# 10XGenomics/supernova

Measured on AMD Instinct MI355X. Metric: Gk-mers/s through count+graph at k=48, 1.2B×150bp; bit-exact counts, higher is better.
Workload: dtype u64

## Files before the change

supernova_amd/csrc/snk_graph.h:

```cpp
#pragma once
#include "snk_ctx.h"
#include "snk_kernels.h"

struct snk_graph_out {
    uint8_t* ctx;
    uint32_t* counts;
    unsigned long long* spectrum;
    uint32_t spectrum_bins;
    uint64_t n_unitigs;
    uint64_t total_bases;
    uint64_t* unitig_off;
    uint8_t* unitig_bases;
    uint32_t* unitig_group;
    uint32_t n_circles;
    uint32_t rank_rounds;
    uint64_t n_boundary;
    uint64_t n_fragments;
};

int snk_graph_sort(snk_ctx* ctx, hipStream_t st, uint32_t K, uint64_t n, snk_u128* keys_in, uint64_t* vals_in,
                   snk_u128* keys_out, uint64_t* vals_out, char* err, size_t errcap);
int snk_graph_build(snk_ctx* ctx, hipStream_t st, uint32_t K, const snk_u128* keys, const uint64_t* vals, uint64_t n,
                    uint32_t do_prune, bool want_unitigs, snk_graph_out* out, char* err, size_t errcap);

// ... 62 lines not shown
                  const uint64_t* boff, const uint8_t* fbases, const uint32_t* fgroup, snk_join_out* out, char* err, size_t errcap);
int snk_dist_answer(snk_ctx* ctx, hipStream_t st, snk_dist_graph* g, const void* d_queries, uint64_t nq, void* d_ans, char* err,
                    size_t errcap);
int snk_dist_apply(snk_ctx* ctx, hipStream_t st, snk_dist_graph* g, const void* d_qbuf, const void* d_ans, uint64_t nq,
                   const unsigned long long* d_qoff, char* err, size_t errcap);
int snk_dist_join(snk_ctx* ctx, hipStream_t st, uint32_t K, uint64_t F, const uint32_t* nk, const unsigned long long* hl_self,
                  const unsigned long long* hl_nb, const uint64_t* boff, const uint8_t* fbases, uint64_t total_fbases,
                  snk_join_out* out, char* err, size_t errcap, const uint32_t* fgroup = nullptr, const uint32_t* sfrag = nullptr,
                  uint64_t n_states = 0, uint32_t* flink_given = nullptr);
int snk_dist_links_query(snk_ctx* ctx, hipStream_t st, bool fill, const snk_frag_out* fr, const unsigned long long* d_node_off, uint32_t world,
                         unsigned long long my_end_base, unsigned long long* d_count_or_cursor, void* d_qbuf, char* err, size_t errcap);
int snk_dist_links_answer(snk_ctx* ctx, hipStream_t st, const snk_frag_out* fr, const void* d_queries, uint64_t nq, unsigned long long my_state_base,
                          uint64_t n_local_states, unsigned long long my_end_base, void* d_ans, char* err, size_t errcap);
int snk_dist_links_apply(snk_ctx* ctx, hipStream_t st, const snk_frag_out* fr, const void* d_qbuf, const void* d_ans, uint64_t nq, uint32_t** flink_out,
                         char* err, size_t errcap);

int snk_dist_links_apply_regions(snk_ctx* ctx, hipStream_t st, const snk_frag_out* fr, const void* d_qbuf, const void* d_ans, uint32_t world, uint64_t cap,
                                 const unsigned long long* counts, uint32_t** flink_out, char* err, size_t errcap);

struct snk_table;
struct snk_bl_state {
    const snk_table* tab;
    uint32_t K, rank, world, NB_total, NBl, do_prune, force_dist;
    uint4* desc;
    uint32_t nchunks, nbig;
    uint32_t* biglist;
    uint8_t *ctx, *pend, *premote;
    uint32_t *counts, *nbr, *rq;
    uint32_t* rq_idx;
    uint16_t* rq_meta;
    unsigned long long* index;
    uint64_t index_mask, n_boundary;
    unsigned long long *qcount, *qcursor;
};
int snk_bl_dist_plan(snk_ctx* ctx, hipStream_t st, snk_bl_state* B, unsigned long long* h_qcount, char* err, size_t errcap);
int snk_bl_dist_fill(snk_ctx* ctx, hipStream_t st, snk_bl_state* B, const unsigned long long* d_qoff, void* d_qbuf, char* err, size_t errcap);
int snk_bl_dist_fragments(snk_ctx* ctx, hipStream_t st, snk_bl_state* B, const unsigned long long* d_node_off, unsigned long long my_node_off,
                          snk_frag_out* out, char* err, size_t errcap);
int snk_local_graph(snk_ctx* ctx, hipStream_t st, uint32_t K, const snk_table* tab, uint32_t do_prune, bool want_unitigs,
                    bool sort_table, bool grouped, snk_graph_out* out, snk_u128** keys_final, float* ms , char* err,
                    size_t errcap);
int snk_spectrum(snk_ctx* ctx, hipStream_t st, const uint32_t* counts, uint64_t n, unsigned long long** bins_out, uint32_t* nbins_out,
                 char* err, size_t errcap);
```

supernova_amd/csrc/snk_graph.hip:

```cpp
#include <string.h>
#include <cstring>
#include <rocprim/rocprim.hpp>

#include "snk_ctx.h"
#include "snk_common.h"
#include "snk_kernels.h"
#include "snk_graph.h"
#include "snk_stages.h"

namespace {

constexpr uint32_t NONE = 0xFFFFFFFFu;
constexpr int TB = 256;

__device__ __forceinline__ snk_kmer load_key(const snk_u128* keys, uint64_t i) {
    const uint64_t* p = reinterpret_cast<const uint64_t*>(keys + i);
    snk_kmer k;
    k.lo = p[0];
    k.hi = p[1];
    return k;
}

__global__ void __launch_bounds__(TB) index_build_kernel(const snk_u128* __restrict__ keys, uint64_t n,
                                                         unsigned long long* __restrict__ tab, uint64_t mask) {
// ... 291 lines not shown
        SNK_HIP_TRY(snk_launch(sorted_check_kernel, snk_blocks(n, 256), 256, 0, st, keys_out, n, bad));
        uint32_t h_bad = 0;
        SNK_HIP_TRY(hipMemcpyAsync(&h_bad, bad, 4, hipMemcpyDeviceToHost, st));
        SNK_HIP_TRY(snk_sync(st));
        if (!h_bad) return SNK_OK;
        if (begin_bit == 0) break;
    }
    return snk_fail(SNK_E_INTERNAL, err, errcap, "retained k-mer table is not strictly ascending after the sort");
}

__global__ void __launch_bounds__(TB) rank_init_w_kernel(const uint32_t* __restrict__ link, const uint32_t* __restrict__ w,
                                                         uint64_t ns, uint32_t* __restrict__ nxt, uint32_t* __restrict__ dist,
                                                         uint32_t* __restrict__ tail) {
    uint64_t s = (uint64_t)blockIdx.x * TB + threadIdx.x;
    if (s >= ns) return;
    uint32_t l = link[s];
    if (l == NONE) { nxt[s] = NONE; dist[s] = 0; tail[s] = (uint32_t)s; }
    else { nxt[s] = l ^ 1u; dist[s] = w[l >> 1]; tail[s] = l ^ 1u; }
}
__global__ void __launch_bounds__(TB) rank_zip_kernel(const uint32_t* __restrict__ dist, const uint32_t* __restrict__ tail, uint64_t ns,
                                                      uint2* __restrict__ rk) {
    uint64_t s = (uint64_t)blockIdx.x * TB + threadIdx.x;
    if (s < ns) rk[s] = make_uint2(dist[s], tail[s]);
}

static int rank_lists_wyllie(snk_ctx* ctx, hipStream_t st, uint32_t* link, uint64_t n, const uint32_t* weights, uint8_t* circ ,
                      const uint2** rk_out, uint32_t* n_circles, uint32_t* rounds,
                      char* err, size_t errcap) {
    const uint64_t ns = 2 * n;
    uint32_t *nxt[2], *dst[2], *tl[2];
    for (int b = 0; b < 2; ++b) { G_ALLOC(nxt[b], uint32_t, ns); G_ALLOC(dst[b], uint32_t, ns); G_ALLOC(tl[b], uint32_t, ns); }
    uint32_t* flags;
    G_ALLOC(flags, uint32_t, 4);
    uint32_t* h_flags = nullptr;
    SNK_HIP_TRY(hipHostMalloc((void**)&h_flags, 16, hipHostMallocDefault));
    int max_rounds = 2;
    while ((1ull << (max_rounds - 1)) < ns) ++max_rounds;
    int cur = 0;
    uint32_t rounds_total = 0;
    for (int attempt = 0; attempt < 2; ++attempt) {
        cur = 0;
        if (weights) SNK_HIP_TRY(snk_launch(rank_init_w_kernel, snk_blocks(ns, TB), TB, 0, st, link, weights, ns, nxt[0], dst[0], tl[0]));
        else SNK_HIP_TRY(snk_launch(rank_init_kernel, snk_blocks(ns, TB), TB, 0, st, link, ns, nxt[0], dst[0], tl[0]));
        bool converged = false;
        for (int r = 0; r < max_rounds; ++r) {
            SNK_HIP_TRY(hipMemsetAsync(flags, 0, 4, st));
            SNK_HIP_TRY(snk_launch(rank_round_kernel, snk_blocks(ns, TB), TB, 0, st, nxt[cur], dst[cur], tl[cur], ns,
                                   nxt[cur ^ 1], dst[cur ^ 1], tl[cur ^ 1], flags));
            cur ^= 1;
            ++rounds_total;
            SNK_HIP_TRY(hipMemcpyAsync(h_flags, flags, 4, hipMemcpyDeviceToHost, st));
            SNK_HIP_TRY(snk_sync(st));
            if (h_flags[0] == 0) { converged = true; break; }
        }
        if (converged) break;
        if (attempt == 1) { (void)hipHostFree(h_flags); return snk_fail(SNK_E_INTERNAL, err, errcap, "unitig ranking did not converge after the circle cut"); }
        uint32_t *jump[2] = {dst[cur ^ 1], tl[cur ^ 1]};
        uint32_t* mn[2];
        G_ALLOC(mn[0], uint32_t, ns);
        G_ALLOC(mn[1], uint32_t, ns);
        SNK_HIP_TRY(snk_launch(cyc_init_kernel, snk_blocks(ns, TB), TB, 0, st, nxt[cur], link, ns, jump[0], mn[0]));
        int c2 = 0;
        for (int r = 0; r < max_rounds; ++r) {
            SNK_HIP_TRY(snk_launch(cyc_round_kernel, snk_blocks(ns, TB), TB, 0, st, jump[c2], mn[c2], ns, jump[c2 ^ 1], mn[c2 ^ 1]));
            c2 ^= 1;
        }
// ... 28 lines not shown
                                                         uint32_t* __restrict__ spl_state) {
    uint64_t s = (uint64_t)blockIdx.x * TB + threadIdx.x;
    if (s >= ns || !spl[s]) return;
    spl_state[sid[s]] = (uint32_t)s;
}
__global__ void __launch_bounds__(TB) spl_pack_kernel(const uint32_t* __restrict__ link, const uint8_t* __restrict__ spl,
                                                      const uint32_t* __restrict__ sid, uint64_t ns, unsigned long long* __restrict__ wrec) {
    uint64_t s = (uint64_t)blockIdx.x * TB + threadIdx.x;
    if (s >= ns) return;
    unsigned long long r = link[s];
    if (spl[s]) r |= ((unsigned long long)sid[s] << 32) | (1ull << 63);
    wrec[s] = r;
}
__global__ void __launch_bounds__(TB) spl_walk1_kernel(const unsigned long long* __restrict__ wrec, const uint32_t* __restrict__ spl_state,
                                                       const uint32_t* __restrict__ w, uint64_t m, uint32_t* __restrict__ rnxt,
                                                       uint32_t* __restrict__ rdist, uint32_t* __restrict__ rtail) {
    uint64_t k = (uint64_t)blockIdx.x * TB + threadIdx.x;
    if (k >= m) return;
    uint32_t cur = spl_state[k];
    unsigned long long rec = wrec[cur];
    uint32_t d = 0, nx = NONE;
    for (;;) {
        uint32_t l = (uint32_t)rec;
        if (l == NONE) { nx = NONE; break; }
        cur = l ^ 1u;
        rec = wrec[cur];
        d += w ? w[cur >> 1] : 1u;
        if (rec >> 63) { nx = (uint32_t)(rec >> 32) & 0x7FFFFFFFu; break; }
    }
    rnxt[k] = nx;
    rdist[k] = d;
    rtail[k] = cur;
}
__global__ void __launch_bounds__(TB) spl_walk2_kernel(const unsigned long long* __restrict__ wrec, const uint32_t* __restrict__ spl_state,
                                                       const uint32_t* __restrict__ w, const uint32_t* __restrict__ rdist,
                                                       const uint32_t* __restrict__ rtail, uint64_t m, uint2* __restrict__ rk) {
    uint64_t k = (uint64_t)blockIdx.x * TB + threadIdx.x;
    if (k >= m) return;
    uint32_t cur = spl_state[k];
    unsigned long long rec = wrec[cur];
    uint32_t d = rdist[k];
    const uint32_t t = rtail[k];
    for (;;) {
        rk[cur] = make_uint2(d, t);
        uint32_t l = (uint32_t)rec;
        if (l == NONE) break;
        cur = l ^ 1u;
        rec = wrec[cur];
        if (rec >> 63) break;
        d -= w ? w[cur >> 1] : 1u;
    }
}
__global__ void __launch_bounds__(TB) unranked_check_kernel(const uint2* __restrict__ rk, uint64_t ns, uint32_t* __restrict__ flag) {
    uint64_t s = (uint64_t)blockIdx.x * TB + threadIdx.x;
    if (s < ns && rk[s].y == NONE) *flag = 1u;
}

__global__ void __launch_bounds__(TB) spl_reach_kernel(const unsigned long long* __restrict__ wrec, const uint32_t* __restrict__ spl_state, uint64_t m,
                                                       uint8_t* __restrict__ reach) {
    const uint64_t k = (uint64_t)blockIdx.x * TB + threadIdx.x;
    if (k >= m) return;
    uint32_t cur = spl_state[k];
    unsigned long long rec = wrec[cur];
    for (;;) {
        reach[cur] = 1;
        const uint32_t l = (uint32_t)rec;
        if (l == NONE) break;
        cur = l ^ 1u;
        rec = wrec[cur];
        if (rec >> 63) break;
    }
}
__global__ void __launch_bounds__(TB) scyc_init_kernel(const uint32_t* __restrict__ rn_final, const uint32_t* __restrict__ rn_orig,
                                                       const uint32_t* __restrict__ spl_state, uint64_t m, uint32_t* __restrict__ jump, uint32_t* __restrict__ mn) {
    const uint64_t k = (uint64_t)blockIdx.x * TB + threadIdx.x;
    if (k >= m) return;
    const bool on = rn_final[k] != NONE;
    jump[k] = on ? rn_orig[k] : NONE;
    mn[k] = on ? spl_state[k] >> 1 : NONE;
}
__device__ __forceinline__ void cut_at(uint32_t* link, uint32_t s, uint8_t* circ, uint32_t* n_cut) {
    const uint32_t partner = link[s];
    link[s] = NONE;
    if (partner != NONE) link[partner] = NONE;
    circ[s] = 1;
    if (partner != NONE) circ[partner] = 1;
    atomicAdd(n_cut, 1u);
}
// ... 43 lines not shown
        SNK_HIP_TRY(snk_launch(scyc_init_kernel, snk_blocks(m, TB), TB, 0, st, rn_final, rn_orig, spl_state, m, jump[0], mn[0]));
        int max_rounds = 2;
        while ((1ull << (max_rounds - 1)) < m + 1) ++max_rounds;
        int c2 = 0;
        for (int r = 0; r < max_rounds; ++r) {
            SNK_HIP_TRY(snk_launch(cyc_round_kernel, snk_blocks(m, TB), TB, 0, st, jump[c2], mn[c2], m, jump[c2 ^ 1], mn[c2 ^ 1]));
            c2 ^= 1;
        }
        SNK_HIP_TRY(snk_launch(scyc_cut_kernel, snk_blocks(m, TB), TB, 0, st, mn[c2], spl_state, m, link, d_flags, circ));
    }
    {
        const uint32_t cap = 1u << 18;
        uint32_t* list;
        G_ALLOC(list, uint32_t, cap);
        SNK_HIP_TRY(snk_launch(free_circle_find_kernel, snk_blocks(ns, TB), TB, 0, st, reach, ns, (const uint32_t*)link, list, cap, d_flags + 2, d_flags + 1));
        SNK_HIP_TRY(snk_launch(cut_list_kernel, cap / TB, TB, 0, st, (const uint32_t*)list, (const uint32_t*)(d_flags + 2), cap, link, d_flags, circ));
    }
    uint32_t h[2] = {0, 0};
    SNK_HIP_TRY(hipMemcpyAsync(h, d_flags, 8, hipMemcpyDeviceToHost, st));
    SNK_HIP_TRY(snk_sync(st));
    *n_cut = h[0];
    *bad = h[1];
    return SNK_OK;
}

static int rank_lists(snk_ctx* ctx, hipStream_t st, uint32_t* link, uint64_t n, const uint32_t* weights, uint8_t* circ ,
                      const uint2** rk_out, uint32_t* n_circles, uint32_t* rounds,
                      char* err, size_t errcap) {
    const uint64_t ns = 2 * n;
    if (ns < 4096 || snk_opt_u32(ctx, SNK_OPT_rank_wyllie))
        return rank_lists_wyllie(ctx, st, link, n, weights, circ, rk_out, n_circles, rounds, err, errcap);
    uint32_t cut_total = 0;
    for (int attempt = 0; attempt < 2; ++attempt) {
    uint8_t* spl;
    uint32_t *flag32, *sid;
    G_ALLOC(spl, uint8_t, ns + 1);
    G_ALLOC(flag32, uint32_t, ns + 1);
    G_ALLOC(sid, uint32_t, ns + 1);
    SNK_HIP_TRY(hipMemsetAsync(flag32 + ns, 0, 4, st));
    const uint32_t split_mask = (1u << snk_opt_u32(ctx, SNK_OPT_split_log2)) - 1u;
    SNK_HIP_TRY(snk_launch(spl_mark_kernel, snk_blocks(ns, TB), TB, 0, st, link, ns, split_mask, spl, flag32));
    {
        size_t tb = 0;
        SNK_HIP_TRY(rocprim::exclusive_scan((void*)nullptr, tb, flag32, sid, 0u, (size_t)(ns + 1), rocprim::plus<uint32_t>(), st));
        void* tmp;
        int rc = snk_ctx_alloc(ctx, tb, &tmp, err, errcap);
        if (rc) return rc;
        SNK_HIP_TRY(rocprim::exclusive_scan(tmp, tb, flag32, sid, 0u, (size_t)(ns + 1), rocprim::plus<uint32_t>(), st));
    }
    uint32_t m32 = 0;
    SNK_HIP_TRY(hipMemcpyAsync(&m32, sid + ns, 4, hipMemcpyDeviceToHost, st));
    SNK_HIP_TRY(snk_sync(st));
    const uint64_t m = m32;
    uint32_t* spl_state = flag32;
    if (m) SNK_HIP_TRY(snk_launch(spl_collect_kernel, snk_blocks(ns, TB), TB, 0, st, spl, sid, ns, spl_state));
    uint32_t *rn[2], *rd[2], *rt[2];
    for (int b = 0; b < 2; ++b) { G_ALLOC(rn[b], uint32_t, m + 1); G_ALLOC(rd[b], uint32_t, m + 1); G_ALLOC(rt[b], uint32_t, m + 1); }
    unsigned long long* wrec;
    G_ALLOC(wrec, unsigned long long, ns);
    SNK_HIP_TRY(snk_launch(spl_pack_kernel, snk_blocks(ns, TB), TB, 0, st, link, spl, sid, ns, wrec));
    SNK_HIP_TRY(snk_launch(spl_walk1_kernel, snk_blocks(m, TB), TB, 0, st, wrec, spl_state, weights, m, rn[0], rd[0], rt[0]));
    uint32_t* rn_orig;
    G_ALLOC(rn_orig, uint32_t, m + 1);
    if (m) SNK_HIP_TRY(hipMemcpyAsync(rn_orig, rn[0], m * 4, hipMemcpyDeviceToDevice, st));
    uint32_t* flags;
    G_ALLOC(flags, uint32_t, 4);
    int max_rounds = 2;
    while ((1ull << (max_rounds - 1)) < m + 1) ++max_rounds;
    int cur = 0;
    uint32_t r_done = 0;
    uint2* rk = nullptr;
    bool converged = false, unranked = false;
    G_ALLOC(rk, uint2, ns);
    const int batch0 = (int)snk_opt_u32(ctx, SNK_OPT_rank_round_batch0);
    for (int r = 0; r < max_rounds && !converged;) {
        const int upto = r == 0 ? (batch0 < max_rounds ? batch0 : max_rounds) : max_rounds;
        SNK_HIP_TRY(hipMemsetAsync(flags, 0, 8, st));
        for (; r < upto; ++r) {
            SNK_HIP_TRY(snk_launch(rank_round_kernel, snk_blocks(m, TB), TB, 0, st, rn[cur], rd[cur], rt[cur], m, rn[cur ^ 1], rd[cur ^ 1], rt[cur ^ 1],
                                   r + 1 == upto ? flags : flags + 2));
            cur ^= 1;
            ++r_done;
        }
        SNK_HIP_TRY(hipMemsetAsync(rk, 0xFF, ns * 8, st));
        SNK_HIP_TRY(snk_launch(spl_walk2_kernel, snk_blocks(m, TB), TB, 0, st, wrec, spl_state, weights, rd[cur], rt[cur], m, rk));
        SNK_HIP_TRY(snk_launch(unranked_check_kernel, snk_blocks(ns, TB), TB, 0, st, rk, ns, flags + 1));
        uint32_t h2[2] = {0, 0};
        SNK_HIP_TRY(hipMemcpyAsync(h2, flags, 8, hipMemcpyDeviceToHost, st));
        SNK_HIP_TRY(snk_sync(st));
        converged = h2[0] == 0;
        unranked = h2[1] != 0;
    }
    if (converged && !unranked) {
        *rk_out = rk;
        *n_circles = cut_total;
        *rounds = r_done;
        return SNK_OK;
    }
    if (!circ || attempt == 1) break;
    uint32_t n_cut = 0, bad = 0;
    int rcc = cut_circles_sparse(ctx, st, link, ns, m, spl_state, wrec, rn_orig, rn[cur], converged, circ, &n_cut, &bad, err, errcap);
    if (rcc) return rcc;
    if (bad || n_cut == 0) break;
    cut_total += n_cut;
    }
    {
        uint32_t nc2 = 0;
        int rcw = rank_lists_wyllie(ctx, st, link, n, weights, circ, rk_out, &nc2, rounds, err, errcap);
        *n_circles = cut_total + nc2;
        return rcw;
    }
}

namespace {
__global__ void __launch_bounds__(TB) spl_walk1p_kernel(const unsigned long long* __restrict__ wrec, const uint32_t* __restrict__ spl_state,
                                                        const uint32_t* __restrict__ w, uint64_t k0, uint64_t cnt, uint4* __restrict__ out) {
    const uint64_t i = (uint64_t)blockIdx.x * TB + threadIdx.x;
    if (i >= cnt) return;
    uint32_t cur = spl_state[k0 + i];
    unsigned long long rec = wrec[cur];
    uint32_t d = 0, nx = NONE, steps = 1;
    for (;;) {
        const uint32_t l = (uint32_t)rec;
        if (l == NONE) { nx = NONE; break; }
        cur = l ^ 1u;
        rec = wrec[cur];
        d += w[cur >> 1];
        if (rec >> 63) { nx = (uint32_t)(rec >> 32) & 0x7FFFFFFFu; break; }
        ++steps;
    }
    out[i] = make_uint4(nx, d, cur, steps);
}
// ... 986 lines not shown
```

supernova_amd/csrc/snk_local.hip:

```cpp
#include <string.h>
#include <cstring>
#include <rocprim/rocprim.hpp>

#include <type_traits>

#include "snk_ctx.h"
#include "snk_common.h"
#include "snk_kernels.h"
#include "snk_graph.h"
#include "snk_stages.h"

namespace {

constexpr uint32_t NONE = 0xFFFFFFFFu;
constexpr unsigned long long NONE64 = ~0ull;
constexpr uint16_t NONE16 = 0xFFFFu;
constexpr int TB = 256;

struct chunk_src {
    const uint32_t* chunk_n;
    const uint32_t* chunk_base;
    const uint4* extra;
    const unsigned long long* region_off;
    uint32_t NB, n_extra, n_regions;
// ... 45 lines not shown
    } else {
        const uint4 e = cs.extra[c - cs.NB];
        bucket = e.x; off = e.y; n = e.z & 0xFFFu; region = e.z >> 12; meta = e.w;
    }
    const uint64_t base = cs.region_off[region] + off;
    desc[c] = make_uint4((uint32_t)base, n, bucket, meta);
    if (desc_src) desc_src[c] = (uint64_t)region * region_cap + off;
}
__device__ __forceinline__ chunk_t chunk_get(const uint4* __restrict__ desc, uint32_t c) {
    const uint4 d = desc[c];
    chunk_t k;
    k.base = d.x; k.n = d.y; k.bucket = d.z; k.lg = d.w >> 24; k.id = d.w & 0xFFFFFFu; k.span = 1;
    if (d.w >> 31) { k.lg = 0; k.id = 0; k.span = d.w & 0xFFFFu; }
    return k;
}

__device__ __forceinline__ snk_kmer load_key(const snk_u128* keys, uint64_t i) {
    const uint64_t* p = reinterpret_cast<const uint64_t*>(keys + i);
    snk_kmer k;
    k.lo = p[0];
    k.hi = p[1];
    return k;
}
__device__ __forceinline__ uint32_t lhash(uint64_t hi, uint64_t lo) {
    uint32_t x = (uint32_t)(hi >> 32) * 0x9E3779B1u ^ (uint32_t)hi * 0x85EBCA77u ^ (uint32_t)(lo >> 32) * 0xC2B2AE3Du ^
                 (uint32_t)lo * 0x27D4EB2Fu;
    return snk_mix32(x);
}
template <int K>
__device__ __forceinline__ uint32_t oriented_base(snk_kmer k, bool rc, int idx) {
    return rc ? (snk_kmer_base<K>(k, K - 1 - idx) ^ 3u) : snk_kmer_base<K>(k, idx);
}

template <int K, int CAP, int T, bool BIG, bool GR, int MM>
__device__ __forceinline__ void bl_prune_chunk(const uint32_t c, const uint4* __restrict__ desc, uint32_t NB, bl_shard sh, const bl_regions& rg,
                                                     const snk_u128* __restrict__ keys, const uint64_t* __restrict__ vals,
                                                     uint32_t do_prune, uint8_t* __restrict__ ctx_out,
                                                     uint32_t* __restrict__ count_out, uint8_t* __restrict__ pend_out,
                                                     uint32_t* __restrict__ nbr_out, uint32_t* __restrict__ nbnd,
                                                     uint32_t* __restrict__ biglist, uint32_t* __restrict__ nbig,
                                                     unsigned long long* __restrict__ gindex, uint64_t gmask) {
    constexpr int HT = CAP <= 256 ? 512 : 4096;
    typedef typename std::conditional<(K <= 48 && !GR), uint32_t, uint64_t>::type klo_w;
    constexpr int KLS = (K <= 48 && !GR) ? 32 : 0;
    __shared__ uint64_t khi[CAP];
    __shared__ klo_w klo[CAP];
    __shared__ uint32_t ht[HT];
    __shared__ uint32_t bcnt;
    const int tid = threadIdx.x;
    const chunk_t ch = chunk_get(desc, c);
    if (ch.n == 0) return;
    if (!BIG && ch.n > (uint32_t)CAP) {
        if (tid == 0) biglist[atomicAdd(nbig, 1u)] = c;
        return;
    }
    const uint32_t n = ch.n;
    uint64_t src = ch.base;
    if (rg.keys_r) { src = rg.desc_src[c]; keys = rg.keys_r; vals = rg.vals_r; }
    __syncthreads();
    for (int s = tid; s < HT; s += T) ht[s] = 0;
    if (tid == 0) bcnt = 0;
    constexpr int NPT = (CAP + T - 1) / T;
    uint64_t myv[NPT];
    snk_kmer kq[NPT];
#pragma unroll
    for (int q = 0; q < NPT; ++q) {
        const uint32_t i = tid + q * T;
        myv[q] = 0;
        if (i < n) {
            kq[q] = load_key(keys, src + i);
            myv[q] = vals[src + i];
        }
    }
#pragma unroll
// ... 100 lines not shown
                uint64_t wn;
                if (bit < 4) {
                    constexpr int pl = K - MM;
                    wn = pl < 32 ? ((y.hi << (2 * pl)) | (y.lo >> (64 - 2 * pl))) : (pl == 32 ? y.lo : (y.lo << (2 * pl - 64)));
                } else wn = y.hi;
                const uint32_t nkey = snk_mmer_key_top<MM>(wn);
                if (nkey < mk) mk = nkey;
                const uint32_t gb = snk_bucket_of_key(mk ^ (GR ? snk_group_mix((uint32_t)ktag) : 0u), NB);
                const uint32_t db = gb - (sh.bucket_base + ch.bucket);
                bool here = ch.span == 1 ? db == 0u : (gb >= sh.bucket_base + ch.bucket && db % sh.G == 0u && db / sh.G < ch.span);
                const bool remote = sh.NBl && gb / sh.NBl != sh.me;
                if (here && ch.lg) {
                    const snk_kmer r = snk_kmer_rc<K>(y);
                    snk_kmer cn = snk_kmer_lt(r, y) ? r : y;
                    if (GR) cn.lo |= ktag;
                    uint32_t h1, h2;
                    snk_kmer_hash_count<(K > 48) || GR>(cn, &h1, &h2);
                    here = (h2 & split_mask) == ch.id;
                }
                if (here && !(do_prune & 2u)) { if (!(do_prune & 1u)) atomicOr(&resL[th], 1u << bit); }
                else atomicOr(&resL[th], (1u << bit) | (0x100u << bit) | (remote ? (0x10000u << bit) : 0u));
            }
        }
        __syncthreads();
        const uint32_t res = resL[tid];
        keep |= res & 0xFFu;
        const uint32_t pm = (res >> 8) & 0xFFu;
        __syncthreads();
        if (!act) continue;
        const uint64_t gi = ch.base + i;
        ctx_out[gi] = (uint8_t)keep;
        pend_out[gi] = (uint8_t)pm;
        if (sh.premote) sh.premote[gi] = (uint8_t)(res >> 16);
        count_out[gi] = (uint32_t)(v >> 8);
        nbr_out[gi] = (nb0 == NONE ? 0x0FFFu : nb0) | (snk_kmer_eq(k, kr) ? 0x8000u : 0u) | ((nb1 == NONE ? 0x0FFFu : nb1) << 16);
        if (pm) {
            ++mybnd;
            if (gindex) {
                snk_kmer kk;
                kk.hi = khi[i];
                kk.lo = (uint64_t)klo[i] << KLS;
                uint32_t h1, h2;
                snk_kmer_hash2(kk, &h1, &h2);
                uint64_t slot = (((uint64_t)h1 << 32) | h2) & gmask;
                const unsigned long long ent = ((unsigned long long)h1 << 32) | (unsigned long long)(gi + 1);
                if (gindex[gmask + 1] == 0ull) {
                    bool placed = false;
                    for (uint32_t tries = 0; tries < 64; ++tries) {
                        const unsigned long long old = atomicCAS(&gindex[slot], 0ull, ent);
                        if (old == 0ull) { placed = true; break; }
                        slot = (slot + 1) & gmask;
                    }
                    if (!placed) gindex[gmask + 1] = 1ull;
                }
            }
        }
    }
    snk_wave_add(&bcnt, mybnd);
    __syncthreads();
    if (tid == 0) nbnd[c] = bcnt;
}
template <int K, int CAP, int T, bool BIG, bool GR, int MM>
__global__ void __launch_bounds__(T) bl_prune_kernel(const uint4* __restrict__ desc, uint32_t NB, bl_shard sh, bl_regions rg, const uint32_t* __restrict__ biglist_in,
                                                     uint32_t nchunks, uint32_t cpw,
                                                     const snk_u128* __restrict__ keys, const uint64_t* __restrict__ vals,
                                                     uint32_t do_prune, uint8_t* __restrict__ ctx_out,
                                                     uint32_t* __restrict__ count_out, uint8_t* __restrict__ pend_out,
                                                     uint32_t* __restrict__ nbr_out, uint32_t* __restrict__ nbnd,
                                                     uint32_t* __restrict__ biglist, uint32_t* __restrict__ nbig, const uint32_t* __restrict__ n_dev,
                                                     unsigned long long* __restrict__ gindex, uint64_t gmask) {
    if (BIG && n_dev) {
        const uint32_t nb = *n_dev;
        for (uint32_t w = blockIdx.x; w < nb; w += gridDim.x)
            bl_prune_chunk<K, CAP, T, BIG, GR, MM>(biglist_in[w], desc, NB, sh, rg, keys, vals, do_prune, ctx_out, count_out, pend_out, nbr_out, nbnd, biglist, nbig, gindex, gmask);
        return;
    }
    for (uint32_t r = 0; r < cpw; ++r) {
        const uint32_t w = blockIdx.x * cpw + r;
        if (w >= nchunks) return;
        bl_prune_chunk<K, CAP, T, BIG, GR, MM>(BIG ? biglist_in[w] : w, desc, NB, sh, rg, keys, vals, do_prune, ctx_out, count_out, pend_out, nbr_out,
                                       nbnd, biglist, nbig, gindex, gmask);
    }
}

__global__ void __launch_bounds__(TB) bl_index_build_kernel(const snk_u128* __restrict__ keys, const uint8_t* __restrict__ pend,
                                                            uint64_t n, unsigned long long* __restrict__ tab, uint64_t mask) {
    const uint64_t i = (uint64_t)blockIdx.x * TB + threadIdx.x;
    if (i >= n || !pend[i]) return;
    const snk_kmer k = load_key(keys, i);
    uint32_t h1, h2;
    snk_kmer_hash2(k, &h1, &h2);
    uint64_t slot = (((uint64_t)h1 << 32) | h2) & mask;
    const unsigned long long ent = ((unsigned long long)h1 << 32) | (unsigned long long)(i + 1);
    for (;;) {
        const unsigned long long old = atomicCAS(&tab[slot], 0ull, ent);
        if (old == 0ull) break;
        slot = (slot + 1) & mask;
    }
}
template <int K, bool GR>
__global__ void __launch_bounds__(TB) bl_resolve_kernel(const snk_u128* __restrict__ keys, const uint8_t* __restrict__ pend,
                                                        uint64_t n, const unsigned long long* __restrict__ tab, uint64_t mask,
                                                        uint32_t do_prune, uint8_t* __restrict__ ctx, uint32_t* __restrict__ rq,
                                                        const uint8_t* __restrict__ premote) {
    constexpr int SPAN = 8 * TB;
    __shared__ uint16_t list[SPAN];
    __shared__ uint32_t cnt;
    const uint64_t base = (uint64_t)blockIdx.x * SPAN;
    if (threadIdx.x == 0) cnt = 0;
    __syncthreads();
    {
        const uint64_t i8 = base + 8ull * threadIdx.x;
        unsigned long long w = 0;
        if (i8 + 8 <= n) w = *reinterpret_cast<const unsigned long long*>(pend + i8);
// ... 470 lines not shown
    uint32_t *nbnd, *ctr;
    G_ALLOC(B->ctx, uint8_t, n + 16);
    G_ALLOC(B->pend, uint8_t, n + 16);
    G_ALLOC(B->counts, uint32_t, n + 4);
    G_ALLOC(B->nbr, uint32_t, n + 2);
    G_ALLOC(B->rq, uint32_t, 2 * n + 2);
    G_ALLOC(nbnd, uint32_t, (uint64_t)nchunks + 1);
    G_ALLOC(B->biglist, uint32_t, n / SCAP + 2);
    G_ALLOC(ctr, uint32_t, 16);
    B->premote = nullptr;
    if (B->world > 1 || B->force_dist) {
        G_ALLOC(B->premote, uint8_t, n + 16);
        SNK_HIP_TRY(hipMemsetAsync(B->premote, 0, n + 16, st));
    }
    SNK_HIP_TRY(hipMemsetAsync(nbnd, 0, ((uint64_t)nchunks + 1) * 4, st));
    SNK_HIP_TRY(hipMemsetAsync(ctr, 0, 64, st));
    bl_shard sh;
    sh.bucket_base = B->premote ? B->rank * B->NBl : 0u;
    sh.NBl = B->premote ? B->NBl : 0u;
    sh.me = B->rank;
    sh.G = tab->n_regions ? tab->n_regions : 1u;
    sh.premote = B->premote;
    const uint32_t NBh = B->premote ? B->NB_total : tab->NB;
    const uint32_t cpw = snk_opt_u32(ctx, SNK_OPT_bl_cpw);
    uint64_t tg0 = 0;
    unsigned long long* index0 = nullptr;
    if (snk_opt_u32(ctx, SNK_OPT_bl_index_fused)) {
        const uint64_t guess = (ctx->last_bnd_n == n && ctx->last_bnd) ? ctx->last_bnd + ctx->last_bnd / 8 : n / 5;
        tg0 = 1024;
        while (tg0 < 2 * guess) tg0 <<= 1;
        G_ALLOC(index0, unsigned long long, tg0 + 1);
        SNK_HIP_TRY(hipMemsetAsync(index0, 0, (tg0 + 1) * 8, st));
    }
    bl_regions rg;
    rg.keys_r = tab->keys_r; rg.vals_r = tab->vals_r; rg.desc_src = desc_src;
    rg.keys_dense = const_cast<snk_u128*>(tab->keys);
    const bool long_m = ctx->mlen == (uint32_t)SNK_M_LONG;
    SNK_HIP_TRY(snk_launch(long_m ? bl_prune_kernel<K, SCAP, ST, false, GR, SNK_M_LONG> : bl_prune_kernel<K, SCAP, ST, false, GR, SNK_M_OF(K)>, snk_blocks(nchunks, cpw), ST, 0, st, (const uint4*)B->desc, NBh, sh, rg,
                           (const uint32_t*)nullptr, nchunks, cpw, tab->keys, tab->vals, B->do_prune | (snk_opt_u32(ctx, SNK_OPT_bl_noclassify) ? 2u : 0u), B->ctx, B->counts, B->pend, B->nbr, nbnd,
                           B->biglist, ctr, (const uint32_t*)nullptr, index0, tg0 - 1));
    uint32_t h_nbig = 0;
    SNK_HIP_TRY(hipMemcpyAsync(ctr + 1, ctr, 4, hipMemcpyDeviceToDevice, st));
    SNK_HIP_TRY(snk_launch(long_m ? bl_prune_kernel<K, BCAP, BT, true, GR, SNK_M_LONG> : bl_prune_kernel<K, BCAP, BT, true, GR, SNK_M_OF(K)>, 2048, BT, 0, st, (const uint4*)B->desc, NBh, sh, rg,
                           (const uint32_t*)B->biglist, 0u, 1u, tab->keys, tab->vals, B->do_prune | (snk_opt_u32(ctx, SNK_OPT_bl_noclassify) ? 2u : 0u), B->ctx, B->counts, B->pend, B->nbr,
                           nbnd, B->biglist, ctr + 2, (const uint32_t*)(ctr + 1), index0, tg0 - 1));
    if (tab->keys_r) {
        snk_ctx_release_block(ctx, tab->keys_r);
        snk_ctx_release_block(ctx, tab->vals_r);
    }
    unsigned long long* d_sum;
    G_ALLOC(d_sum, unsigned long long, 2);
    {
        size_t tb = 0;
        auto in = rocprim::make_transform_iterator(nbnd, [] __device__(uint32_t v) { return (unsigned long long)v; });
        SNK_HIP_TRY(rocprim::reduce((void*)nullptr, tb, in, d_sum, 0ull, (size_t)nchunks, rocprim::plus<unsigned long long>(), st));
        void* tmp;
        int rc = snk_ctx_alloc(ctx, tb, &tmp, err, errcap);
        if (rc) return rc;
        SNK_HIP_TRY(rocprim::reduce(tmp, tb, in, d_sum, 0ull, (size_t)nchunks, rocprim::plus<unsigned long long>(), st));
    }
    unsigned long long h_bnd = 0, h_gaveup = 0;
    if (index0) SNK_HIP_TRY(hipMemcpyAsync(&h_gaveup, index0 + tg0, 8, hipMemcpyDeviceToHost, st));
    SNK_HIP_TRY(hipMemcpyAsync(&h_bnd, d_sum, 8, hipMemcpyDeviceToHost, st));
    SNK_HIP_TRY(hipMemcpyAsync(&h_nbig, ctr + 1, 4, hipMemcpyDeviceToHost, st));
    SNK_HIP_TRY(snk_sync(st));
    B->nbig = h_nbig;
    B->n_boundary = h_bnd;
    ctx->last_bnd = h_bnd; ctx->last_bnd_n = n;
    uint64_t tg = 1024;
    while (tg < 2 * h_bnd) tg <<= 1;
    const bool fused_ok = index0 && !h_gaveup && h_bnd * 4 <= tg0 * 3;
    if (fused_ok) { B->index = index0; tg = tg0; }
    else {
        if (index0) snk_ctx_release_block(ctx, index0);
        G_ALLOC(B->index, unsigned long long, tg);
        SNK_HIP_TRY(hipMemsetAsync(B->index, 0, tg * 8, st));
    }
    B->index_mask = tg - 1;
    if (h_bnd) {
        if (!fused_ok) SNK_HIP_TRY(snk_launch(bl_index_build_kernel, snk_blocks(n, TB), TB, 0, st, tab->keys, B->pend, n, B->index, tg - 1));
        SNK_HIP_TRY(snk_launch(bl_resolve_kernel<K, GR>, snk_blocks(n, 8 * TB), TB, 0, st, tab->keys, B->pend, n,
                               B->index, tg - 1, B->do_prune, B->ctx, B->rq, (const uint8_t*)B->premote));
    }
    return SNK_OK;
}

template <int K, bool DIST, bool GR>
static int bl_fragments_impl(snk_ctx* ctx, hipStream_t st, snk_bl_state* B, const bl_dist_args& da, snk_frag_out* out, char* err,
                             size_t errcap) {
    const snk_table* tab = B->tab;
    const uint32_t nchunks = B->nchunks, h_nbig = B->nbig;
    uint32_t *nfrag, *foff;
    uint64_t *nbases, *boff;
    G_ALLOC(nfrag, uint32_t, (uint64_t)nchunks + 1);
    G_ALLOC(foff, uint32_t, (uint64_t)nchunks + 1);
    G_ALLOC(nbases, uint64_t, (uint64_t)nchunks + 1);
    G_ALLOC(boff, uint64_t, (uint64_t)nchunks + 1);
    SNK_HIP_TRY(hipMemsetAsync(nfrag, 0, ((uint64_t)nchunks + 1) * 4, st));
    bl_extra_pool xp0;
// ... 60 lines not shown
}

template <int K, bool GR>
static int local_graph_impl(snk_ctx* ctx, hipStream_t st, const snk_table* tab, uint32_t do_prune, bool want_unitigs,
                            bool sort_table, snk_graph_out* out, snk_u128** keys_final, float* ms, char* err, size_t errcap) {
    memset(out, 0, sizeof *out);
    const uint64_t n = tab->n;
    *keys_final = tab->keys;
    if (n == 0) {
        int rc0 = snk_spectrum(ctx, st, nullptr, 0, &out->spectrum, &out->spectrum_bins, err, errcap);
        if (rc0) return rc0;
        G_ALLOC(out->unitig_off, uint64_t, 2);
        SNK_HIP_TRY(hipMemsetAsync(out->unitig_off, 0, 16, st));
        G_ALLOC(out->unitig_bases, uint8_t, 16);
        G_ALLOC(out->ctx, uint8_t, 16);
        G_ALLOC(out->counts, uint32_t, 4);
        return SNK_OK;
    }
    if (n >= (1ull << 31)) return snk_fail(SNK_E_UNSUPPORTED, err, errcap, "more than 2^31 retained k-mers on one GPU (%llu)", (unsigned long long)n);
#ifndef SNK_DBG_NO_CHUNK_CHECK
    if (snk_count_slots(K) > (uint32_t)BCAP + 768u + 64u)
#else
    if (false)
#endif
        return snk_fail(SNK_E_INTERNAL, err, errcap, "bucket-local graph: chunk capacity %d is below the count table's limit", BCAP);
    snk_phase_timer tm(st);
    tm.mark();
    snk_bl_state B;
    memset(&B, 0, sizeof B);
    B.tab = tab;
    B.K = K;
    B.world = 1;
    B.do_prune = do_prune;
    int rc = bl_prune_impl<K, GR>(ctx, st, &B, err, errcap);
    if (rc) return rc;
    tm.mark();
    tm.mark();
    out->n_boundary = B.n_boundary;
    if (want_unitigs) {
        snk_frag_out fo;
        memset(&fo, 0, sizeof fo);
        bl_dist_args da;
        memset(&da, 0, sizeof da);
        if ((rc = bl_fragments_impl<K, false, GR>(ctx, st, &B, da, &fo, err, errcap))) return rc;
        tm.mark();
        snk_join_out jo;
        rc = snk_dist_join(ctx, st, K, fo.n_frags, fo.nk, fo.hl_self, fo.hl_nb, fo.boff, fo.bases, fo.total_bases, &jo, err, errcap, fo.fgroup, fo.sfrag, 2 * n);
        if (rc) return rc;
        tm.mark();
        out->n_unitigs = jo.n_unitigs;
        out->total_bases = jo.total_bases;
        out->unitig_off = jo.unitig_off;
        out->unitig_bases = jo.unitig_bases;
        out->unitig_group = jo.unitig_group;
        out->n_circles = jo.n_circles;
        out->rank_rounds = jo.rank_rounds;
        out->n_fragments = fo.n_frags;
    } else {
        G_ALLOC(out->unitig_off, uint64_t, 2);
        SNK_HIP_TRY(hipMemsetAsync(out->unitig_off, 0, 16, st));
        G_ALLOC(out->unitig_bases, uint8_t, 16);
        tm.mark();
        tm.mark();
    }
    out->ctx = B.ctx;
    out->counts = B.counts;
    if (sort_table) {
        uint64_t *v_in, *v_out;
        snk_u128* k_out;
        G_ALLOC(v_in, uint64_t, n + 1);
        G_ALLOC(v_out, uint64_t, n + 1);
        G_ALLOC(k_out, snk_u128, n + 1);
        SNK_HIP_TRY(snk_launch(bl_pack_vals_kernel, snk_blocks(n, TB), TB, 0, st, B.counts, B.ctx, n, v_in));
        rc = snk_graph_sort(ctx, st, K, n, tab->keys, v_in, k_out, v_out, err, errcap);
        if (rc) return rc;
        SNK_HIP_TRY(snk_launch(bl_unpack_vals_kernel, snk_blocks(n, TB), TB, 0, st, v_out, n, B.counts, B.ctx));
        *keys_final = k_out;
    }
    if ((rc = snk_spectrum(ctx, st, B.counts, n, &out->spectrum, &out->spectrum_bins, err, errcap))) return rc;
    tm.mark();
    if (ms) { ms[0] = tm.ms(0, 1); ms[1] = tm.ms(1, 2); ms[2] = tm.ms(2, 3); ms[3] = tm.ms(3, 4); ms[4] = tm.ms(4, 5); }
    return SNK_OK;
}

int snk_local_graph(snk_ctx* ctx, hipStream_t st, uint32_t K, const snk_table* tab, uint32_t do_prune, bool want_unitigs,
                    bool sort_table, bool grouped, snk_graph_out* out, snk_u128** keys_final, float* ms, char* err, size_t errcap) {
    if (tab->sorted) return snk_fail(SNK_E_INTERNAL, err, errcap, "bucket-local graph needs the table in chunk order");
    if (grouped) {
        if (K != 48) return snk_fail(SNK_E_UNSUPPORTED, err, errcap, "grouped graphs need K=48");
        return local_graph_impl<48, true>(ctx, st, tab, do_prune, want_unitigs, sort_table, out, keys_final, ms, err, errcap);
    }
    if (K == 48) return local_graph_impl<48, false>(ctx, st, tab, do_prune, want_unitigs, sort_table, out, keys_final, ms, err, errcap);
    if (K == 60) return local_graph_impl<60, false>(ctx, st, tab, do_prune, want_unitigs, sort_table, out, keys_final, ms, err, errcap);
    return snk_fail(SNK_E_UNSUPPORTED, err, errcap, "K=%u is not supported (48 or 60)", K);
}

int snk_bl_dist_plan(snk_ctx* ctx, hipStream_t st, snk_bl_state* B, unsigned long long* h_qcount, char* err, size_t errcap) {
    B->force_dist = 1;
    const uint64_t n = B->tab->n;
    G_ALLOC(B->qcount, unsigned long long, B->world + 4);
    G_ALLOC(B->qcursor, unsigned long long, B->world + 1);
    G_ALLOC(B->rq_idx, uint32_t, 2 * n + 2);
    G_ALLOC(B->rq_meta, uint16_t, 2 * n + 2);
    SNK_HIP_TRY(hipMemsetAsync(B->qcount, 0, (B->world + 1) * 8ull, st));
    SNK_HIP_TRY(hipMemsetAsync(B->rq_idx, 0xFF, (2 * n + 2) * 4, st));
    if (h_qcount) for (uint32_t r = 0; r < B->world; ++r) h_qcount[r] = 0;
    if (n == 0) {
        G_ALLOC(B->ctx, uint8_t, 16);
        G_ALLOC(B->counts, uint32_t, 4);
        G_ALLOC(B->index, unsigned long long, 1024);
        SNK_HIP_TRY(hipMemsetAsync(B->index, 0, 1024 * 8, st));
        B->index_mask = 1023;
// ... 51 lines not shown
```

Measured before the change: 98.38.

## Fuse spectrum histogram into prune kernel and streamline sparse list ranking

Builds the count spectrum inside the prune kernel using per-block LDS bins plus replicated global bins, which removes the separate snk_spectrum pass over counts. Separately, the sparse list-ranking path drops its mark, collect and pack kernels and the flag array in favour of a transform-iterator scan and one setup kernel. It also pairs each list with its mate so walk2 writes both strands at once, which replaces the rk memset and the unranked-check kernel with an atomic count. The rn_orig copy is now recomputed only on the circle-cut fallback. Risks are extra atomics in the prune kernel, a fixed 65536-bin spectrum with an overflow fallback, and more complex mate-pairing logic.

Result: faster. 100.0, median of 6 (+1.7%).

```diff
diff --git a/supernova_amd/csrc/snk_graph.h b/supernova_amd/csrc/snk_graph.h
--- a/supernova_amd/csrc/snk_graph.h
+++ b/supernova_amd/csrc/snk_graph.h
@@ -118,6 +118,8 @@
     unsigned long long* index;
     uint64_t index_mask, n_boundary;
     unsigned long long *qcount, *qcursor;
+    unsigned long long* spec;
+    uint32_t want_spec, spec_over;
 };
 int snk_bl_dist_plan(snk_ctx* ctx, hipStream_t st, snk_bl_state* B, unsigned long long* h_qcount, char* err, size_t errcap);
 int snk_bl_dist_fill(snk_ctx* ctx, hipStream_t st, snk_bl_state* B, const unsigned long long* d_qoff, void* d_qbuf, char* err, size_t errcap);
diff --git a/supernova_amd/csrc/snk_graph.hip b/supernova_amd/csrc/snk_graph.hip
--- a/supernova_amd/csrc/snk_graph.hip
+++ b/supernova_amd/csrc/snk_graph.hip
@@ -347,6 +347,7 @@
     for (int b = 0; b < 2; ++b) { G_ALLOC(nxt[b], uint32_t, ns); G_ALLOC(dst[b], uint32_t, ns); G_ALLOC(tl[b], uint32_t, ns); }
     uint32_t* flags;
     G_ALLOC(flags, uint32_t, 4);
+    SNK_HIP_TRY(hipMemsetAsync(flags, 0, 16, st));
     uint32_t* h_flags = nullptr;
     SNK_HIP_TRY(hipHostMalloc((void**)&h_flags, 16, hipHostMallocDefault));
     int max_rounds = 2;
@@ -441,28 +442,80 @@
     rdist[k] = d;
     rtail[k] = cur;
 }
-__global__ void __launch_bounds__(TB) spl_walk2_kernel(const unsigned long long* __restrict__ wrec, const uint32_t* __restrict__ spl_state,
-                                                       const uint32_t* __restrict__ w, const uint32_t* __restrict__ rdist,
-                                                       const uint32_t* __restrict__ rtail, uint64_t m, uint2* __restrict__ rk) {
-    uint64_t k = (uint64_t)blockIdx.x * TB + threadIdx.x;
-    if (k >= m) return;
-    uint32_t cur = spl_state[k];
-    unsigned long long rec = wrec[cur];
-    uint32_t d = rdist[k];
-    const uint32_t t = rtail[k];
-    for (;;) {
-        rk[cur] = make_uint2(d, t);
-        uint32_t l = (uint32_t)rec;
-        if (l == NONE) break;
-        cur = l ^ 1u;
-        rec = wrec[cur];
-        if (rec >> 63) break;
-        d -= w ? w[cur >> 1] : 1u;
-    }
-}
 __global__ void __launch_bounds__(TB) unranked_check_kernel(const uint2* __restrict__ rk, uint64_t ns, uint32_t* __restrict__ flag) {
     uint64_t s = (uint64_t)blockIdx.x * TB + threadIdx.x;
     if (s < ns && rk[s].y == NONE) *flag = 1u;
+}
+
+struct spl_flag_fn {
+    const uint32_t* link;
+    uint64_t ns;
+    uint32_t split_mask;
+    __device__ uint32_t operator()(uint64_t s) const {
+        if (s >= ns) return 0u;
+        return (link[s ^ 1ull] == NONE || sampled_state((uint32_t)s, split_mask)) ? 1u : 0u;
+    }
+};
+__global__ void __launch_bounds__(TB) spl_setup_kernel(const uint32_t* __restrict__ link, const uint32_t* __restrict__ sid, uint64_t ns, uint32_t split_mask,
+                                                       uint32_t* __restrict__ spl_state, unsigned long long* __restrict__ wrec) {
+    uint64_t s = (uint64_t)blockIdx.x * TB + threadIdx.x;
+    if (s >= ns) return;
+    unsigned long long r = link[s];
+    if (link[s ^ 1ull] == NONE || sampled_state((uint32_t)s, split_mask)) {
+        const uint32_t id = sid[s];
+        r |= ((unsigned long long)id << 32) | (1ull << 63);
+        spl_state[id] = (uint32_t)s;
+    }
+    wrec[s] = r;
+}
+__global__ void __launch_bounds__(TB) spl_head_info_kernel(const unsigned long long* __restrict__ wrec, const uint32_t* __restrict__ spl_state,
+                                                           const uint32_t* __restrict__ w, const uint32_t* __restrict__ rdist,
+                                                           const uint32_t* __restrict__ rtail, uint64_t m, uint2* __restrict__ info) {
+    const uint64_t k = (uint64_t)blockIdx.x * TB + threadIdx.x;
+    if (k >= m) return;
+    const uint32_t h = spl_state[k];
+    if ((uint32_t)wrec[h ^ 1u] != NONE) return;
+    const uint32_t t = rtail[k];
+    const uint32_t id = (uint32_t)(wrec[t ^ 1u] >> 32) & 0x7FFFFFFFu;
+    info[id] = make_uint2(h, rdist[k] + (w ? w[h >> 1] : 1u));
+}
+__global__ void __launch_bounds__(TB) spl_walk2m_kernel(const unsigned long long* __restrict__ wrec, const uint32_t* __restrict__ spl_state,
+                                                        const uint32_t* __restrict__ w, const uint32_t* __restrict__ rdist,
+                                                        const uint32_t* __restrict__ rtail, const uint2* __restrict__ info, uint64_t m,
+                                                        uint2* __restrict__ rk, uint32_t* __restrict__ ranked) {
+    const uint64_t k = (uint64_t)blockIdx.x * TB + threadIdx.x;
+    uint32_t cnt = 0;
+    if (k < m) {
+        uint32_t cur = spl_state[k];
+        unsigned long long rec = wrec[cur];
+        uint32_t d = rdist[k];
+        const uint32_t t = rtail[k];
+        const uint2 hw = info[(uint32_t)(wrec[t ^ 1u] >> 32) & 0x7FFFFFFFu];
+        const uint32_t mt = hw.x ^ 1u;
+        if (t <= mt) {
+            const bool self = t == mt;
+            uint32_t wc = w ? w[cur >> 1] : 1u;
+            for (;;) {
+                if (self) {
+                    rk[cur] = make_uint2(d, t);
+                    cnt += 1;
+                } else {
+                    const uint32_t dm = hw.y - d - wc;
+                    ((uint4*)rk)[cur >> 1] = (cur & 1u) ? make_uint4(dm, mt, d, t) : make_uint4(d, t, dm, mt);
+                    cnt += 2;
+                }
+                const uint32_t l = (uint32_t)rec;
+                if (l == NONE) break;
+                cur = l ^ 1u;
+                rec = wrec[cur];
+                if (rec >> 63) break;
+                wc = w ? w[cur >> 1] : 1u;
+                d -= wc;
+            }
+        }
+    }
+    for (int o = 32; o > 0; o >>= 1) cnt += __shfl_xor(cnt, o);
+    if ((threadIdx.x & 63) == 0 && cnt) atomicAdd(ranked, cnt);
 }
 
 __global__ void __launch_bounds__(TB) spl_reach_kernel(const unsigned long long* __restrict__ wrec, const uint32_t* __restrict__ spl_state, uint64_t m,
@@ -572,37 +625,32 @@
         return rank_lists_wyllie(ctx, st, link, n, weights, circ, rk_out, n_circles, rounds, err, errcap);
     uint32_t cut_total = 0;
     for (int attempt = 0; attempt < 2; ++attempt) {
-    uint8_t* spl;
-    uint32_t *flag32, *sid;
-    G_ALLOC(spl, uint8_t, ns + 1);
-    G_ALLOC(flag32, uint32_t, ns + 1);
+    uint32_t* sid;
     G_ALLOC(sid, uint32_t, ns + 1);
-    SNK_HIP_TRY(hipMemsetAsync(flag32 + ns, 0, 4, st));
     const uint32_t split_mask = (1u << snk_opt_u32(ctx, SNK_OPT_split_log2)) - 1u;
-    SNK_HIP_TRY(snk_launch(spl_mark_kernel, snk_blocks(ns, TB), TB, 0, st, link, ns, split_mask, spl, flag32));
     {
+        auto flag_it = rocprim::make_transform_iterator(rocprim::counting_iterator<uint64_t>(0), spl_flag_fn{link, ns, split_mask});
         size_t tb = 0;
-        SNK_HIP_TRY(rocprim::exclusive_scan((void*)nullptr, tb, flag32, sid, 0u, (size_t)(ns + 1), rocprim::plus<uint32_t>(), st));
+        SNK_HIP_TRY(rocprim::exclusive_scan((void*)nullptr, tb, flag_it, sid, 0u, (size_t)(ns + 1), rocprim::plus<uint32_t>(), st));
         void* tmp;
         int rc = snk_ctx_alloc(ctx, tb, &tmp, err, errcap);
         if (rc) return rc;
-        SNK_HIP_TRY(rocprim::exclusive_scan(tmp, tb, flag32, sid, 0u, (size_t)(ns + 1), rocprim::plus<uint32_t>(), st));
+        SNK_HIP_TRY(rocprim::exclusive_scan(tmp, tb, flag_it, sid, 0u, (size_t)(ns + 1), rocprim::plus<uint32_t>(), st));
     }
     uint32_t m32 = 0;
     SNK_HIP_TRY(hipMemcpyAsync(&m32, sid + ns, 4, hipMemcpyDeviceToHost, st));
     SNK_HIP_TRY(snk_sync(st));
     const uint64_t m = m32;
-    uint32_t* spl_state = flag32;
-    if (m) SNK_HIP_TRY(snk_launch(spl_collect_kernel, snk_blocks(ns, TB), TB, 0, st, spl, sid, ns, spl_state));
+    uint32_t* spl_state;
+    G_ALLOC(spl_state, uint32_t, m + 1);
     uint32_t *rn[2], *rd[2], *rt[2];
     for (int b = 0; b < 2; ++b) { G_ALLOC(rn[b], uint32_t, m + 1); G_ALLOC(rd[b], uint32_t, m + 1); G_ALLOC(rt[b], uint32_t, m + 1); }
     unsigned long long* wrec;
     G_ALLOC(wrec, unsigned long long, ns);
-    SNK_HIP_TRY(snk_launch(spl_pack_kernel, snk_blocks(ns, TB), TB, 0, st, link, spl, sid, ns, wrec));
+    SNK_HIP_TRY(snk_launch(spl_setup_kernel, snk_blocks(ns, TB), TB, 0, st, (const uint32_t*)link, (const uint32_t*)sid, ns, split_mask, spl_state, wrec));
     SNK_HIP_TRY(snk_launch(spl_walk1_kernel, snk_blocks(m, TB), TB, 0, st, wrec, spl_state, weights, m, rn[0], rd[0], rt[0]));
-    uint32_t* rn_orig;
-    G_ALLOC(rn_orig, uint32_t, m + 1);
-    if (m) SNK_HIP_TRY(hipMemcpyAsync(rn_orig, rn[0], m * 4, hipMemcpyDeviceToDevice, st));
+    uint2* info;
+    G_ALLOC(info, uint2, m + 1);
     uint32_t* flags;
     G_ALLOC(flags, uint32_t, 4);
     int max_rounds = 2;
@@ -622,14 +670,13 @@
             cur ^= 1;
             ++r_done;
         }
-        SNK_HIP_TRY(hipMemsetAsync(rk, 0xFF, ns * 8, st));
-        SNK_HIP_TRY(snk_launch(spl_walk2_kernel, snk_blocks(m, TB), TB, 0, st, wrec, spl_state, weights, rd[cur], rt[cur], m, rk));
-        SNK_HIP_TRY(snk_launch(unranked_check_kernel, snk_blocks(ns, TB), TB, 0, st, rk, ns, flags + 1));
+        SNK_HIP_TRY(snk_launch(spl_head_info_kernel, snk_blocks(m, TB), TB, 0, st, wrec, spl_state, weights, rd[cur], rt[cur], m, info));
+        SNK_HIP_TRY(snk_launch(spl_walk2m_kernel, snk_blocks(m, TB), TB, 0, st, wrec, spl_state, weights, rd[cur], rt[cur], (const uint2*)info, m, rk, flags + 1));
         uint32_t h2[2] = {0, 0};
         SNK_HIP_TRY(hipMemcpyAsync(h2, flags, 8, hipMemcpyDeviceToHost, st));
         SNK_HIP_TRY(snk_sync(st));
         converged = h2[0] == 0;
-        unranked = h2[1] != 0;
+        unranked = h2[1] != ns;
     }
     if (converged && !unranked) {
         *rk_out = rk;
@@ -638,6 +685,11 @@
         return SNK_OK;
     }
     if (!circ || attempt == 1) break;
+    uint32_t *rn_orig, *rd_spare, *rt_spare;
+    G_ALLOC(rn_orig, uint32_t, m + 1);
+    G_ALLOC(rd_spare, uint32_t, m + 1);
+    G_ALLOC(rt_spare, uint32_t, m + 1);
+    SNK_HIP_TRY(snk_launch(spl_walk1_kernel, snk_blocks(m, TB), TB, 0, st, wrec, spl_state, weights, m, rn_orig, rd_spare, rt_spare));
     uint32_t n_cut = 0, bad = 0;
     int rcc = cut_circles_sparse(ctx, st, link, ns, m, spl_state, wrec, rn_orig, rn[cur], converged, circ, &n_cut, &bad, err, errcap);
     if (rcc) return rcc;
diff --git a/supernova_amd/csrc/snk_local.hip b/supernova_amd/csrc/snk_local.hip
--- a/supernova_amd/csrc/snk_local.hip
+++ b/supernova_amd/csrc/snk_local.hip
@@ -101,6 +101,17 @@
     return rc ? (snk_kmer_base<K>(k, K - 1 - idx) ^ 3u) : snk_kmer_base<K>(k, idx);
 }
 
+constexpr int BL_SPEC_LDS = 128;
+constexpr int BL_SPEC_REPL = 64;
+constexpr uint32_t BL_SPEC_BINS = 65536u;
+constexpr uint32_t BL_SPEC_OVER = BL_SPEC_BINS + BL_SPEC_REPL * BL_SPEC_LDS / 2;
+constexpr uint32_t BL_SPEC_WORDS = BL_SPEC_OVER + 16;
+__global__ void __launch_bounds__(BL_SPEC_LDS) bl_spec_fold_kernel(unsigned long long* __restrict__ spec) {
+    const uint32_t* rep = reinterpret_cast<const uint32_t*>(spec + BL_SPEC_BINS);
+    unsigned long long s = 0;
+    for (int r = 0; r < BL_SPEC_REPL; ++r) s += rep[r * BL_SPEC_LDS + threadIdx.x];
+    spec[threadIdx.x] += s;
+}
 template <int K, int CAP, int T, bool BIG, bool GR, int MM>
 __device__ __forceinline__ void bl_prune_chunk(const uint32_t c, const uint4* __restrict__ desc, uint32_t NB, bl_shard sh, const bl_regions& rg,
                                                      const snk_u128* __restrict__ keys, const uint64_t* __restrict__ vals,
@@ -108,7 +119,8 @@
                                                      uint32_t* __restrict__ count_out, uint8_t* __restrict__ pend_out,
                                                      uint32_t* __restrict__ nbr_out, uint32_t* __restrict__ nbnd,
                                                      uint32_t* __restrict__ biglist, uint32_t* __restrict__ nbig,
-                                                     unsigned long long* __restrict__ gindex, uint64_t gmask) {
+                                                     unsigned long long* __restrict__ gindex, uint64_t gmask,
+                                                     unsigned long long* __restrict__ spec, uint32_t* __restrict__ shist) {
     constexpr int HT = CAP <= 256 ? 512 : 4096;
     typedef typename std::conditional<(K <= 48 && !GR), uint32_t, uint64_t>::type klo_w;
     constexpr int KLS = (K <= 48 && !GR) ? 32 : 0;
@@ -275,7 +287,14 @@
         ctx_out[gi] = (uint8_t)keep;
         pend_out[gi] = (uint8_t)pm;
         if (sh.premote) sh.premote[gi] = (uint8_t)(res >> 16);
-        count_out[gi] = (uint32_t)(v >> 8);
+        const uint32_t cnt = (uint32_t)(v >> 8);
+        count_out[gi] = cnt;
+        if (spec) {
+            const uint32_t sc = cnt > 0xFFFFFFu ? 0xFFFFFFu : cnt;
+            if (sc < (uint32_t)BL_SPEC_LDS) atomicAdd(&shist[sc], 1u);
+            else if (sc < BL_SPEC_BINS) atomicAdd(&spec[sc], 1ull);
+            else spec[BL_SPEC_OVER] = 1ull;
+        }
         nbr_out[gi] = (nb0 == NONE ? 0x0FFFu : nb0) | (snk_kmer_eq(k, kr) ? 0x8000u : 0u) | ((nb1 == NONE ? 0x0FFFu : nb1) << 16);
         if (pm) {
             ++mybnd;
@@ -311,18 +330,30 @@
                                                      uint32_t* __restrict__ count_out, uint8_t* __restrict__ pend_out,
                                                      uint32_t* __restrict__ nbr_out, uint32_t* __restrict__ nbnd,
                                                      uint32_t* __restrict__ biglist, uint32_t* __restrict__ nbig, const uint32_t* __restrict__ n_dev,
-                                                     unsigned long long* __restrict__ gindex, uint64_t gmask) {
+                                                     unsigned long long* __restrict__ gindex, uint64_t gmask, unsigned long long* __restrict__ spec) {
+    __shared__ uint32_t shist[BL_SPEC_LDS];
+    if (spec) {
+        for (int j = threadIdx.x; j < BL_SPEC_LDS; j += T) shist[j] = 0;
+        __syncthreads();
+    }
     if (BIG && n_dev) {
         const uint32_t nb = *n_dev;
         for (uint32_t w = blockIdx.x; w < nb; w += gridDim.x)
-            bl_prune_chunk<K, CAP, T, BIG, GR, MM>(biglist_in[w], desc, NB, sh, rg, keys, vals, do_prune, ctx_out, count_out, pend_out, nbr_out, nbnd, biglist, nbig, gindex, gmask);
-        return;
-    }
-    for (uint32_t r = 0; r < cpw; ++r) {
-        const uint32_t w = blockIdx.x * cpw + r;
-        if (w >= nchunks) return;
-        bl_prune_chunk<K, CAP, T, BIG, GR, MM>(BIG ? biglist_in[w] : w, desc, NB, sh, rg, keys, vals, do_prune, ctx_out, count_out, pend_out, nbr_out,
-                                       nbnd, biglist, nbig, gindex, gmask);
+            bl_prune_chunk<K, CAP, T, BIG, GR, MM>(biglist_in[w], desc, NB, sh, rg, keys, vals, do_prune, ctx_out, count_out, pend_out, nbr_out, nbnd, biglist, nbig, gindex, gmask,
+                                                   spec, shist);
+    } else {
+        for (uint32_t r = 0; r < cpw; ++r) {
+            const uint32_t w = blockIdx.x * cpw + r;
+            if (w >= nchunks) break;
+            bl_prune_chunk<K, CAP, T, BIG, GR, MM>(BIG ? biglist_in[w] : w, desc, NB, sh, rg, keys, vals, do_prune, ctx_out, count_out, pend_out, nbr_out,
+                                           nbnd, biglist, nbig, gindex, gmask, spec, shist);
+        }
+    }
+    if (spec) {
+        __syncthreads();
+        uint32_t* rep = reinterpret_cast<uint32_t*>(spec + BL_SPEC_BINS) + (blockIdx.x % BL_SPEC_REPL) * BL_SPEC_LDS;
+        for (int j = threadIdx.x; j < BL_SPEC_LDS; j += T)
+            if (shist[j]) atomicAdd(&rep[j], shist[j]);
     }
 }
 
@@ -859,18 +890,24 @@
         G_ALLOC(index0, unsigned long long, tg0 + 1);
         SNK_HIP_TRY(hipMemsetAsync(index0, 0, (tg0 + 1) * 8, st));
     }
+    unsigned long long* spec = nullptr;
+    if (B->want_spec) {
+        G_ALLOC(spec, unsigned long long, BL_SPEC_WORDS);
+        SNK_HIP_TRY(hipMemsetAsync(spec, 0, (size_t)BL_SPEC_WORDS * 8, st));
+    }
     bl_regions rg;
     rg.keys_r = tab->keys_r; rg.vals_r = tab->vals_r; rg.desc_src = desc_src;
     rg.keys_dense = const_cast<snk_u128*>(tab->keys);
     const bool long_m = ctx->mlen == (uint32_t)SNK_M_LONG;
     SNK_HIP_TRY(snk_launch(long_m ? bl_prune_kernel<K, SCAP, ST, false, GR, SNK_M_LONG> : bl_prune_kernel<K, SCAP, ST, false, GR, SNK_M_OF(K)>, snk_blocks(nchunks, cpw), ST, 0, st, (const uint4*)B->desc, NBh, sh, rg,
                            (const uint32_t*)nullptr, nchunks, cpw, tab->keys, tab->vals, B->do_prune | (snk_opt_u32(ctx, SNK_OPT_bl_noclassify) ? 2u : 0u), B->ctx, B->counts, B->pend, B->nbr, nbnd,
-                           B->biglist, ctr, (const uint32_t*)nullptr, index0, tg0 - 1));
+                           B->biglist, ctr, (const uint32_t*)nullptr, index0, tg0 - 1, spec));
     uint32_t h_nbig = 0;
     SNK_HIP_TRY(hipMemcpyAsync(ctr + 1, ctr, 4, hipMemcpyDeviceToDevice, st));
     SNK_HIP_TRY(snk_launch(long_m ? bl_prune_kernel<K, BCAP, BT, true, GR, SNK_M_LONG> : bl_prune_kernel<K, BCAP, BT, true, GR, SNK_M_OF(K)>, 2048, BT, 0, st, (const uint4*)B->desc, NBh, sh, rg,
                            (const uint32_t*)B->biglist, 0u, 1u, tab->keys, tab->vals, B->do_prune | (snk_opt_u32(ctx, SNK_OPT_bl_noclassify) ? 2u : 0u), B->ctx, B->counts, B->pend, B->nbr,
-                           nbnd, B->biglist, ctr + 2, (const uint32_t*)(ctr + 1), index0, tg0 - 1));
+                           nbnd, B->biglist, ctr + 2, (const uint32_t*)(ctr + 1), index0, tg0 - 1, spec));
+    if (spec) SNK_HIP_TRY(snk_launch(bl_spec_fold_kernel, 1, BL_SPEC_LDS, 0, st, spec));
     if (tab->keys_r) {
         snk_ctx_release_block(ctx, tab->keys_r);
         snk_ctx_release_block(ctx, tab->vals_r);
@@ -886,12 +923,15 @@
         if (rc) return rc;
         SNK_HIP_TRY(rocprim::reduce(tmp, tb, in, d_sum, 0ull, (size_t)nchunks, rocprim::plus<unsigned long long>(), st));
     }
-    unsigned long long h_bnd = 0, h_gaveup = 0;
+    unsigned long long h_bnd = 0, h_gaveup = 0, h_spec_over = 0;
     if (index0) SNK_HIP_TRY(hipMemcpyAsync(&h_gaveup, index0 + tg0, 8, hipMemcpyDeviceToHost, st));
+    if (spec) SNK_HIP_TRY(hipMemcpyAsync(&h_spec_over, spec + BL_SPEC_OVER, 8, hipMemcpyDeviceToHost, st));
     SNK_HIP_TRY(hipMemcpyAsync(&h_bnd, d_sum, 8, hipMemcpyDeviceToHost, st));
     SNK_HIP_TRY(hipMemcpyAsync(&h_nbig, ctr + 1, 4, hipMemcpyDeviceToHost, st));
     SNK_HIP_TRY(snk_sync(st));
     B->nbig = h_nbig;
+    B->spec = spec;
+    B->spec_over = h_spec_over != 0;
     B->n_boundary = h_bnd;
     ctx->last_bnd = h_bnd; ctx->last_bnd_n = n;
     uint64_t tg = 1024;
@@ -1018,6 +1058,7 @@
     B.K = K;
     B.world = 1;
     B.do_prune = do_prune;
+    B.want_spec = sort_table ? 0u : 1u;
     int rc = bl_prune_impl<K, GR>(ctx, st, &B, err, errcap);
     if (rc) return rc;
     tm.mark();
@@ -1063,7 +1104,10 @@
         SNK_HIP_TRY(snk_launch(bl_unpack_vals_kernel, snk_blocks(n, TB), TB, 0, st, v_out, n, B.counts, B.ctx));
         *keys_final = k_out;
     }
-    if ((rc = snk_spectrum(ctx, st, B.counts, n, &out->spectrum, &out->spectrum_bins, err, errcap))) return rc;
+    if (B.spec && !B.spec_over) {
+        out->spectrum = B.spec;
+        out->spectrum_bins = BL_SPEC_BINS;
+    } else if ((rc = snk_spectrum(ctx, st, B.counts, n, &out->spectrum, &out->spectrum_bins, err, errcap))) return rc;
     tm.mark();
     if (ms) { ms[0] = tm.ms(0, 1); ms[1] = tm.ms(1, 2); ms[2] = tm.ms(2, 3); ms[3] = tm.ms(3, 4); ms[4] = tm.ms(4, 5); }
     return SNK_OK;
```
